# DTUWindEnergy/WindGym

Hardware: AMD Instinct MI355X
Metric: env-steps/sec (whole node), 16-turbine farm x 4096 envs (higher is better)
Workload: dtype f32

## Files before the change

windgym_amd/csrc/wg_api.hip:

```cpp
#include <hip/hip_runtime.h>

#include <algorithm>
#include <cmath>
#include <cstdio>
#include <cstdlib>
#include <cstring>
#include <memory>
#include <mutex>
#include <string>
#include <vector>

#include "wg_plan.h"
#include "wg_steady.h"
#include "wg_policy.h"
#include "wg_internal.h"

static const char* wg_hook(const char* name) {
    static const bool on = [] { const char* v = getenv("WG_DEBUG_HOOKS"); return v && v[0] == '1' && v[1] == 0; }();
    if (!on) return nullptr;
    const char* v = getenv(name);
    if (v) {
        static std::string seen;
        static std::mutex seen_mu;
        std::lock_guard<std::mutex> lock(seen_mu);
        const std::string tag = std::string(name) + "=" + v + ";";
        if (seen.find(tag) == std::string::npos) {
            seen += tag;
            fprintf(stderr, "[windgym] WG_DEBUG_HOOKS: %s=%s\n", name, v);
        }
    }
    return v;
}
static WgHooks wg_hooks_read() {
    WgHooks k;
    const auto num = [](const char* name) { WgHookInt r; if (const char* v = wg_hook(name)) { r.set = true; r.v = atoi(v); } return r; };
    k.flow_block = num("WG_FLOW_BLOCK"); k.flow_res = num("WG_FLOW_RES"); k.flow_env = num("WG_FLOW_ENV");
    k.env_wpe = num("WG_ENV_WPE"); k.env_split = num("WG_ENV_SPLIT"); k.step_fused = num("WG_STEP_FUSED");
    k.sums = num("WG_SUMS"); k.lds_pad = num("WG_LDS_PAD"); k.lf_cap = num("WG_LF_CAP"); k.pstride_pad = num("WG_PSTRIDE_PAD");
    k.step_graph = num("WG_STEP_GRAPH");
    k.first_obs_gl_only = wg_hook("WG_FIRST_OBS_GL_ONLY") != nullptr;
    k.no_box8 = wg_hook("WG_NO_BOX8") != nullptr;
    k.debug = wg_hook("WG_DEBUG") != nullptr;
    if (const char* v = wg_hook("WG_TIMELINE_OUT")) { k.timeline = true; k.timeline_out = v; }
    return k;
}

static thread_local std::string g_err;
static int fail(int code, const std::string& msg) {
    g_err = msg;
    return code;
}
extern "C" int wg_set_last_error_(int code, const char* msg) { return fail(code, msg ? msg : ""); }
#define HIPCHK(x)                                                                                   \
    do {                                                                                            \
        hipError_t _e = (x);                                                                        \
        if (_e != hipSuccess)                                                                       \
            return fail(WG_ERR_HIP, std::string(#x) + ": " + hipGetErrorString(_e));                \
    } while (0)

struct Alloc {
    void* ptr;
    size_t bytes;
};

struct wg_env_s {
    WgPlan plan;
    WgHooks hooks;
    WgParams p;
    WgPtrs d;
    FlowP fp;
    FlowPtrs fd;
    unsigned long long flow_steps_mark = 0, particles_mark = 0, added_mark = 0;
    double added_per_launch = 0.0;
    long n_step_launches = 0;
    void* box4 = nullptr;
    void* box4c = nullptr;
    int* box_ids_dev = nullptr;
    void* abox4 = nullptr;
    void* box8 = nullptr;
    void* abox8 = nullptr;
    double* wind_dev = nullptr;
    int device;
    std::vector<Alloc> allocs;
    std::vector<size_t> state_idx;
    uint8_t* mask_dev = nullptr;
    uint64_t* seeds_dev = nullptr;
    bool timing = false;
    int timing_period = 1, timing_phase = 0;
    std::vector<hipEvent_t> ev;
    std::vector<int> ev_kind;
    size_t ev_used = 0;
    struct StepGraph {
// ... 168 lines not shown
    g.rotor_dy = d.rotor_dy; g.rotor_dz = d.rotor_dz;
    g.gp = h->p_dev; g.gd = h->d_dev; g.env_rw = d.env;
    g.roff = d.roff; g.qown = d.qown; g.status = d.status;
}

static void apply_step_path(wg_env_s* h) {
    wg_plan_step_path(h->plan, h->fp.box_cells, (long long)h->fp.anx * h->fp.any * h->fp.anz, &h->fp.envw, &h->fp.env_fused);
}

extern "C" int wg_create(const wg_config* c, int device, wg_handle* out) {
    if (!c || !out) return fail(WG_ERR_INVALID, "null argument");
    std::string err;
    if (int rc = wg_validate_config(c, &err)) return fail(rc, err);
    HIPCHK(hipSetDevice(device));
    int lds_limit = 65536;
    {
        int v = 0;
        if (hipDeviceGetAttribute(&v, hipDeviceAttributeMaxSharedMemoryPerBlock, device) == hipSuccess && v > 0)
            lds_limit = std::min(v, 65536);
    }
    std::unique_ptr<wg_env_s, HandleGuard> owner(new wg_env_s());
    wg_env_s* h = owner.get();
    h->device = device;
    h->hooks = wg_hooks_read();
    if (int rc = wg_plan_create(c, h->hooks, lds_limit, &h->plan, &err)) return fail(rc, err);
    h->p = h->plan.p;
    h->fp = h->plan.f;
    apply_step_path(h);

    if (int rc = create_alloc(h)) return rc;
    if (int rc = create_upload(h, c)) return rc;
    if (int rc = create_alloc_record(h)) return rc;
    create_flow_ptrs(h);
    if (h->hooks.timeline) {
        long long* dbgp = nullptr;
        if (!dev_alloc(h, &dbgp, (size_t)h->p.B * 2 * h->p.F * 16, false)) h->fd.dbg = dbgp;
    }
    wg_launch_create(&h->p, &h->d, nullptr);
    if (sync_dev_params(h)) return WG_ERR_HIP;
    {
        hipError_t e = hipDeviceSynchronize();
        if (e == hipSuccess) e = hipStreamCreateWithFlags(&h->cap_stream, hipStreamNonBlocking);
        if (e != hipSuccess) return fail(WG_ERR_HIP, std::string("wg_create: ") + hipGetErrorString(e));
    }
    if (h->hooks.step_graph.set) h->graph_mode = h->hooks.step_graph.v != 0;
    if (h->hooks.debug) {
        const FlowP& f = h->fp;
        fprintf(stderr, "[windgym] k_flow variant: %s%s, %d threads, LDS %d B per workgroup, slot stride %d floats\n",
                f.envw ? (f.turb_mode == WG_TURB_NONE ? "compact rings / pair-major, one wave per env (k_flow_env)" : "compact rings / sample-major, one wave per env (k_flow_envb)")
                       : (f.res ? "compact rings / pair-major" : "uniform rings / sample-major"),
                f.envw && f.env_split ? " + a pass wave for the running episode's context" : "",
                f.block, f.envw ? f.env_lds : f.lds_bytes, f.pstride);
        fprintf(stderr, "[windgym] plan: res %d block %d gl %d rec_il %d target_chunk %d lf_cap %d lds_bytes %d | envw %d env_wpe %d env_split %d env_fused %d "
                        "env_lds %d env_off_tab %d | sums_mode %d first_obs %d reset_launches %d\n",
                f.res, f.block, f.gl, f.rec_il, f.target_chunk, f.lf_cap, f.lds_bytes, f.envw, f.env_wpe, f.env_split, f.env_fused, f.env_lds,
                f.env_off_tab, h->p.sums_mode, h->plan.first_obs, h->plan.reset_launches);
    }
    *out = owner.release();
    return 0;
}

extern "C" int wg_destroy(wg_handle h) {
    if (!h) return 0;
    hipSetDevice(h->device);
    hipDeviceSynchronize();
    if (h->fd.dbg && h->hooks.timeline) {
        const size_t n = (size_t)h->p.B * 2 * h->p.F * 16;
        std::vector<long long> host(n);
        if (hipMemcpy(host.data(), h->fd.dbg, n * sizeof(long long), hipMemcpyDeviceToHost) == hipSuccess) {
            if (FILE* f = fopen(h->hooks.timeline_out.c_str(), "wb")) { fwrite(host.data(), sizeof(long long), n, f); fclose(f); }
        }
    }
    drop_step_graphs(h);
    if (h->cap_stream) hipStreamDestroy(h->cap_stream);
    for (auto& e : h->ev) hipEventDestroy(e);
    for (auto& a : h->allocs) hipFree(a.ptr);
    if (h->box4) hipFree(h->box4);
    if (h->box4c) hipFree(h->box4c);
    if (h->abox4) hipFree(h->abox4);
    if (h->box8) hipFree(h->box8);
    if (h->abox8) hipFree(h->abox8);
    delete h;
    return 0;
}

extern "C" int wg_obs_dim(wg_handle h, int* obs_dim, int* obs_dim_multi) {
    if (!h) return fail(WG_ERR_INVALID, "null handle");
    if (obs_dim) *obs_dim = h->p.obs_dim;
    if (obs_dim_multi) *obs_dim_multi = h->p.obs_dim_multi;
    return 0;
}
extern "C" int wg_hist_max(wg_handle h, int* hist_max) {
    if (!h || !hist_max) return fail(WG_ERR_INVALID, "null argument");
    *hist_max = h->p.hist_max;
    return 0;
}

static int build_stencil_records(wg_env_s* h, void** owned, const float4** kernel_ptr, const void* box4, int n_boxes, int nx, int ny, int nz) {
    *kernel_ptr = nullptr;
    if (!(h->fp.envw && h->fp.turb_mode != WG_TURB_NONE)) return 0;
    const auto skip = [h](const char* why) {
        if (h->hooks.debug) fprintf(stderr, "[windgym] stencil records not built (%s): k_flow_envb reads the brick-ordered box\n", why);
        return 0;
    };
    if (wg_hooks_read().no_box8) return skip("WG_NO_BOX8");
    const size_t n_cells = (size_t)nx * ny * nz, bytes = n_cells * 128 * (size_t)n_boxes;
    size_t free_b = 0, total_b = 0;
    if (hipMemGetInfo(&free_b, &total_b) != hipSuccess) return skip("hipMemGetInfo failed");
    if (n_cells >= ((size_t)1 << 28)) return skip("a box of 2^28 cells or more");
// ... 725 lines not shown
```

windgym_amd/csrc/wg_env.hip:

```cpp
#include <hip/hip_runtime.h>

#ifndef WG_ENV_ABLATE
#define WG_ENV_ABLATE 0
#endif
#include "wg_env_common.h"
#include "wg_internal.h"

struct __attribute__((aligned(16))) EnvSlotLds {
    int dev_rem, fill_rem, sub, budget;
    double s_new;
    int n_emit, n_valid, new_valid;
    unsigned n_emitted;
    float s_off_f, near_f, move_max, ti_pow;
    double s_off, ws;
    float ws_f, ti_f, wd_env, base_acc;
    int n_pushed, pend_farm_n, pend_base_n, n_flow;
    double c_time;
    int c_head;
    unsigned c_part, c_flow, c_istep, c_tag, n_emitted0;
    float out_pw;
    unsigned c_add;
    int bg_init;
    int pad_[3];
};
static_assert(sizeof(EnvSlotLds) == WG_ENV_SLOT_LDS_BYTES, "keep WG_ENV_SLOT_LDS_BYTES in sync (wg_flow.h)");
#define WG_ENV_OFF_SRC4 0
#define WG_ENV_OFF_REC4 1024
#define WG_ENV_OFF_RING 2048
#define WG_ENV_OFF_XR 3072
#define WG_ENV_OFF_SRC2 3584
#define WG_ENV_OFF_SL 4096
#define WG_ENV_OFF_HDR (WG_ENV_OFF_SL + 4 * WG_ENV_SLOT_LDS_BYTES)
#define WG_ENV_OFF_STAGE (WG_ENV_OFF_HDR + 128)
static_assert(WG_ENV_OFF_STAGE == WG_ENV_FIXED_LDS_BYTES, "keep WG_ENV_FIXED_LDS_BYTES in sync (wg_flow.h)");

__device__ __forceinline__ float env_slot_sums(const float v, const int N, const int NS, const int k, const int tid) {
    if (N == 16) return wg_row_sum(v);
    if (N < 16) {
        const int r = tid >> 4, i = tid & 15;
        const float x = __shfl(v, (r * N + i) & 63, 64);
        const float s = wg_row_sum((i < N && r < NS) ? x : 0.f);
        return __shfl(s, k << 4, 64);
    }
    const int h = tid >> 5, i = tid & 31;
    const float x = __shfl(v, (h * N + i) & 63, 64);
    float s = (i < N && h < NS) ? x : 0.f;
    WG_ROW_REDUCE(s, wg_addf)
    s += __shfl_xor(s, 16, 64);
    return __shfl(s, k << 5, 64);
}

template <bool NOISE, int WPE, int GLUE, int SPLIT>
__device__ __forceinline__ void env_flow(char* const smem, char* const smem_pass, float* const zone, const int wv, const int role, const int mode,
                                         const float* __restrict__ actions, const uint8_t* __restrict__ mask, const int chunk, EnvFlowOut& out) {
    const int tid = threadIdx.x & 63, e = blockIdx.x;
    int N, F, NS, NL;
    float inv_N;
    {
        const KArgsPtr ka = wg_cold_args();
        N = ka->p.N; F = ka->p.F; inv_N = ka->p.inv_N;
        NS = WPE == 2 ? F : 2 * F; NL = NS * N;
    }
    const int kbase = WPE == 2 ? wv * F : 0;
    const bool valid = tid < NL;
    const int g = valid ? tid : 0;
    const int k = (int)(((float)g + 0.5f) * inv_N);
    const int t = g - k * N;
    const int c = WPE == 2 ? wv : (F == 2 ? (k >> 1) : k), farm = F == 2 ? (k & 1) : 0;

    float4* const Lsrc4 = reinterpret_cast<float4*>(smem + WG_ENV_OFF_SRC4);
    uint4* const Lrec4 = reinterpret_cast<uint4*>(smem + WG_ENV_OFF_REC4);
    int4* const Lring = reinterpret_cast<int4*>(smem + WG_ENV_OFF_RING);
    double* const Lxr = reinterpret_cast<double*>(smem + WG_ENV_OFF_XR);
    float2* const Lsrc2 = reinterpret_cast<float2*>(smem + WG_ENV_OFF_SRC2);
    EnvSlotLds* const SL = reinterpret_cast<EnvSlotLds*>(smem + WG_ENV_OFF_SL);
    float* const def = reinterpret_cast<float*>(smem + WG_ENV_OFF_STAGE);
    float* const tiav = def + WG_ENV_CAP;
    unsigned short* const cl = reinterpret_cast<unsigned short*>(tiav + WG_ENV_CAP);
    unsigned short* const ql = reinterpret_cast<unsigned short*>(smem + WG_ENV_OFF_STAGE);
    EnvSlotLds& my = SL[k];

    WG_STAMP(0);
    typedef const __attribute__((address_space(4))) WgEnv* CEnvPtr;
    int env_live;
    bool role_live = false, role_dev = false, defer_init = false, split_on = false;
    float yaw, tu, tti, oyaw;
    {
        const KArgsPtr k0 = wg_cold_args();
        static_assert(sizeof(WgEnv) == 128, "the env header is loaded as 32 words");
        const int hw = reinterpret_cast<const int*>(k0->d.env + e)[tid & 31];
        if (GLUE != 0 && tid < 32) reinterpret_cast<int*>(smem + WG_ENV_OFF_HDR)[tid] = hw;
        out.bg_init_pending = 0; out.rounds = 0; out.first_obs = 0;
        const bool use_mask = mode == WG_MODE_RESET && mask != nullptr;
        const uint8_t mask_byte = *(use_mask ? mask + e : reinterpret_cast<const uint8_t*>(k0->d.env + e));
        const bool masked_out = use_mask && mask_byte == 0;
        const unsigned ctx_id = (unsigned)(e * 2 + c), slot_id = (unsigned)(e * 2 * F + kbase + k);
        const unsigned tb = (unsigned)((e * 2 * F + kbase) * N + g);
        const unsigned tcx = ctx_id * (unsigned)N + (unsigned)t;

        int dev_rem, fill_rem, n_pushed, pend_farm_n, pend_base_n, init_pending, time_max_c, n_valid, c_head;
        unsigned n_emitted, c_part, c_flow, c_istep, c_tag, c_add;
        double s_off, ws, l_xr, l_yr, c_time;
        float ti_f, wd_env, l_yaw, l_u, l_ti, l_act;
        float4 l_bnd;
        int l_roff, l_rnext;
        auto load_state = [&]() __attribute__((always_inline)) {
            const KArgsPtr kl = wg_cold_args();
            const WgSlot& slot = kl->d.slot[slot_id];
            const WgCtx& cx = kl->d.ctx[ctx_id];
            dev_rem = slot.dev_remaining; fill_rem = slot.fill_remaining;
            s_off = slot.s_off; c_time = slot.time; c_head = slot.head; n_valid = slot.n_valid; c_istep = slot.istep;
            n_emitted = slot.n_emitted; c_part = slot.part_count; c_flow = slot.flow_count; c_add = slot.add_count;
            ws = cx.ws; ti_f = (float)cx.ti; wd_env = (float)cx.wd;
            n_pushed = cx.n_pushed; pend_farm_n = cx.pend_farm_n; pend_base_n = cx.pend_base_n;
            c_tag = (unsigned)cx.episode_tag; init_pending = cx.init_pending; time_max_c = cx.time_max;
            const int* ro = kl->d.roff + ctx_id * (unsigned)(N + 1);
            l_roff = ro[(unsigned)t]; l_rnext = ro[(unsigned)t + 1u];
            l_xr = kl->d.xr[tcx]; l_yr = kl->d.yr[tcx];
            l_yaw = kl->d.yaw[tb]; l_u = kl->d.u[tb]; l_ti = kl->d.ti_loc[tb];
            l_bnd = reinterpret_cast<const float4*>(kl->d.bnd)[tb];
        };
        load_state();
        const int n_tab = k0->p.n_tab, S = k0->p.S;
        const unsigned i_tab = (unsigned)min(tid, n_tab - 1), i_s = (unsigned)min(tid, S - 1);
        const float pf_tp = k0->d.tab_power[i_tab], pf_tc = k0->d.tab_ct[i_tab];
        const float pf_dy = k0->d.rotor_dy[i_s], pf_dz = k0->d.rotor_dz[i_s];
        {
            const bool has_act = mode == WG_MODE_STEP && farm == 0;
            const float a = *(has_act ? actions + (unsigned)(e * N + t) : k0->d.tab_ct);
            l_act = has_act ? a : 0.f;
        }

#define WG_HDR_I(f) __builtin_amdgcn_readlane(hw, (int)(offsetof(WgEnv, f) / 4))
        env_live = WG_HDR_I(live);
        int env_done = WG_HDR_I(done), env_shadow_iters = WG_HDR_I(shadow_iters), env_steps_done = WG_HDR_I(steps_done);
        int env_timestep = WG_HDR_I(timestep), env_time_max_live = WG_HDR_I(time_max_live);
#undef WG_HDR_I
        if (SPLIT && role == 1) {
            if (tid == 0) { *reinterpret_cast<int*>(smem + WG_ENV_OFF_HDR) = 0; if (GLUE != 0 && (SPLIT == 1 || wv == 0)) reinterpret_cast<int*>(zone)[LEAN_PRE_FLAG] = 0; }
            asm volatile("s_waitcnt vmcnt(0) lgkmcnt(0)" ::: "memory");
        }
        if (WPE == 2) {
            asm volatile("" : "+s"(env_live), "+s"(env_done), "+s"(env_shadow_iters), "+s"(env_steps_done), "+s"(env_timestep), "+s"(env_time_max_live) : : "memory");
            asm volatile("s_barrier" ::: "memory");
        }
        if (SPLIT && role == 1 && GLUE != 0 && c == env_live) {
            const EnvKArgsPtr kz = (EnvKArgsPtr)wg_cold_args();
            const WgParams& zp = *(const WgParams*)&kz->gp;
            const WgPtrs& zd = *(const WgPtrs*)&kz->gd;
#define WG_HDR_Z(f) __builtin_amdgcn_readlane(hw, (int)(offsetof(WgEnv, f) / 4))
            const int z_np = WG_HDR_Z(n_pushed_live), z_fn = WG_HDR_Z(farm_pow_n), z_bn = WG_HDR_Z(base_pow_n);
#undef WG_HDR_Z
            const int PA = zp.power_avg;
            const SumsRaw zr = wg_sums_load<false, false>(zp, zd, e, e * 2 + env_live, tid < N ? tid : 0, z_np);
            const float z_fo = zd.farm_pow[(size_t)e * PA + z_fn % PA];
            const float z_bo = F == 2 ? zd.base_pow[(size_t)e * PA + z_bn % PA] : 0.f;
            const float z_met = tid < WG_N_METRICS ? zd.metrics[(size_t)e * WG_N_METRICS + tid] : 0.f;
            double* const zs = reinterpret_cast<double*>(zone);
#pragma unroll
            for (int sI = 0; sI < WG_N_CH; ++sI) { zs[LEAN_PRE_S(sI, tid)] = zr.S[sI]; zone[LEAN_PRE_LV(sI, tid)] = zr.lv[sI]; }
            zone[LEAN_PRE_MET(tid)] = z_met;
            if (tid == 0) { zone[LEAN_PRE_FOLD] = z_fo; zone[LEAN_PRE_BOLD] = z_bo; }
            asm volatile("s_waitcnt lgkmcnt(0)" ::: "memory");
            if (tid == 0) env_flag_set(reinterpret_cast<int*>(zone) + LEAN_PRE_FLAG);
        }
        out.env_live = env_live;
        out.truncates = env_timestep >= env_time_max_live;
        out.steps_done = env_steps_done; out.time_max_live = env_time_max_live;

        const bool is_live_c = (c == env_live);
        const int autoreset = k0->p.autoreset;
        int budget = 0;
        if (mode == WG_MODE_STEP) {
            role_live = is_live_c && !env_done;
            role_dev = !is_live_c && autoreset != 0;
            const int bg_pending = WPE == 2 ? (is_live_c ? 0 : __shfl(init_pending, 0, 64)) : __shfl(init_pending, (env_live ^ 1) * F * N, 64);
            out.bg_init_pending = autoreset && bg_pending;
            if (SPLIT == 2 && role == 1 && out.bg_init_pending) return;
            if (autoreset && bg_pending && WPE == 1 && !out.truncates) {
                defer_init = true;
                budget = 0;
            } else if (autoreset && bg_pending) {
                const KArgsPtr ki = wg_cold_args();
                const WgParams& gp = *ki->d.gp;
                env_init_episode<GLUE != 0>(e, env_live ^ 1, tid);
                full_barrier<64>();
                load_state();
                const int fill_max = F == 2 ? max(gp.fill_a, gp.fill_b) : gp.fill_a;
                const int inc = 1 + (gp.extra_inc ? 1 : 0);
                const int tm = WPE == 2 ? ki->d.ctx[e * 2 + env_live].time_max : __shfl(time_max_c, env_live * F * N, 64);
                const long total = (long)((tm + inc - 1) / inc) + 1;
                const int dev0 = __shfl(dev_rem, WPE == 2 ? 0 : (env_live ^ 1) * F * N, 64);
                budget = wg_shadow_share(dev0 + gp.K * fill_max, total - env_steps_done, env_steps_done, e);
                budget = wg_shadow_share(dev_rem + gp.K * fill_rem, total - env_steps_done, env_steps_done, e, farm ? 0x80000000u : 0u);
            } else {
                const int inc = k0->p.env_inc;
                const long total = (long)((env_time_max_live + inc - 1) / inc) + 1;
                budget = role_dev ? wg_shadow_share(dev_rem + k0->p.K * fill_rem, total - env_steps_done, env_steps_done, e, farm ? 0x80000000u : 0u) : 0;
            }
        } else {
            role_dev = is_live_c && !masked_out;
            budget = chunk;
        }
        if (SPLIT) {
            const bool two = valid && role_dev && budget >= 2;
            split_on = mode == WG_MODE_STEP && k0->p.K == 1 && (is_live_c || (SPLIT == 2 && !out.bg_init_pending)) && !defer_init && !__ballot(two);
            if (role == 1 && !split_on) return;
        }
        if (WPE == 2 && valid && t == 0) {
            my.dev_rem = dev_rem; my.fill_rem = fill_rem; my.bg_init = out.bg_init_pending; my.n_flow = 0; my.out_pw = 0.f;
        }
        {
            const bool any_work = valid && (role_live || (role_dev && budget > 0 && (dev_rem > 0 || fill_rem > 0)));
            if (!__ballot(any_work)) {
                if (WPE == 2 && mode == WG_MODE_STEP && !is_live_c && autoreset && role == 0) {
                    const int d0 = __shfl(dev_rem, 0, 64), f0 = __shfl(fill_rem, 0, 64), np0 = __shfl(n_pushed, 0, 64);
                    const KArgsPtr kf = wg_cold_args();
                    if (d0 == 0 && f0 == 0 && kf->d.gd->next_obs_ok != nullptr && kf->d.gd->next_obs_ok[ctx_id] == 0) {
                        out.first_obs = 1;
                        env_first_obs<GLUE != 0>((int)ctx_id, np0, tid);
                    }
                }
                return;
            }
        }

        const KArgsPtr k1 = wg_cold_args();
        const int rlen = l_rnext - l_roff;
        const int head = n_emitted == 0u ? rlen - 1 : fast_mod((int)(n_emitted - 1u), rlen, __builtin_amdgcn_rcpf((float)rlen));
        const float ws_f = (float)ws;
        if (valid) {
            Lxr[g] = l_xr;
            Lsrc4[g] = make_float4((float)l_xr, (float)l_yr, l_bnd.y, l_bnd.z);
            Lsrc2[g] = make_float2(l_bnd.x, l_bnd.w);
            Lring[g] = make_int4(l_roff, rlen, head, k);
            Lrec4[g] = make_uint4(0u, 0u, 0u, __float_as_uint(1.f));
            if (t == 0) {
                my.dev_rem = dev_rem; my.fill_rem = fill_rem; my.sub = 0; my.budget = budget;
                my.n_valid = n_valid; my.n_emitted = n_emitted; my.n_emitted0 = n_emitted;
                my.move_max = fabsf(k1->p.hill) * ws_f * k1->p.dt; my.ti_pow = fast_pow(ti_f, k1->p.tic);
                my.s_off = s_off; my.ws = ws; my.ws_f = ws_f; my.ti_f = ti_f; my.wd_env = wd_env; my.base_acc = 0.f;
                my.n_pushed = n_pushed; my.pend_farm_n = pend_farm_n; my.pend_base_n = pend_base_n; my.n_flow = 0;
                my.bg_init = out.bg_init_pending;
                my.c_time = c_time; my.c_head = c_head; my.c_part = c_part; my.c_flow = c_flow; my.c_istep = c_istep; my.c_tag = c_tag; my.c_add = c_add;
            }
        }
        float* const tabp = reinterpret_cast<float*>(smem + k1->p.env_off_tab);
        float* const tabct = tabp + n_tab;
        float2* const rpt = reinterpret_cast<float2*>(tabct + n_tab);
        const float hub = k1->p.hub;
        auto rp = [&](const float dy_, const float dz_) __attribute__((always_inline)) {
            const float dz = hub + dz_ - hub;
            return make_float2(dy_, dz * dz);
        };
        if (tid < n_tab) { tabp[tid] = pf_tp; tabct[tid] = pf_tc; }
        if (tid < S) rpt[tid] = rp(pf_dy, pf_dz);
        for (int i = tid + 64; i < n_tab; i += 64) { tabp[i] = k1->d.tab_power[i]; tabct[i] = k1->d.tab_ct[i]; }
        for (int i = tid + 64; i < S; i += 64) rpt[i] = rp(k1->d.rotor_dy[i], k1->d.rotor_dz[i]);

        yaw = l_yaw; tu = l_u; tti = l_ti; oyaw = l_yaw;
        if (role_live && farm == 0 && valid) {
            const float a = l_act, ymin = k1->p.yaw_min, ymax = k1->p.yaw_max, ystep = k1->p.yaw_step;
            if (k1->p.action_method == WG_ACT_YAW) {
                yaw = fminf(fmaxf(yaw + a * ystep, ymin), ymax);
            } else {
                float tf = a + 1.0f;
                tf = tf * 0.5f;
                tf = tf * (ymax - ymin);
                tf = tf + ymin;
                const float ny = fminf(fmaxf(tf, yaw - ystep), yaw + ystep);
                yaw = fminf(fmaxf(ny, ymin), ymax);
            }
        }
    }
    float tpow = 0.f, tct = 0.f, cg = 1.f;
    float sws = 0.f, swd = 0.f, syaw = 0.f, sp_ = 0.f;
    int part_acc = 0, stream_acc = 0;
    bool stepped = false;
    lds_barrier<64>();
    WG_STAMP(1);

    for (int round = 0;; ++round) {
        bool stepping, is_dev;
        int sub, K;
        {
            const KArgsPtr kr = wg_cold_args();
            K = kr->p.K;
            const int4 sch = *reinterpret_cast<const int4*>(&my.dev_rem);
            const bool active = sch.x > 0 || sch.y > 0;
            stepping = valid && (role_live ? (round < K) : (role_dev && active && (sch.w > 0 || sch.z != 0)));
            is_dev = !role_live && sch.x > 0;
            sub = sch.z;
            if (!__ballot(stepping)) break;
        out.rounds = round + 1;
            if (round > 0) full_barrier<64>();

            if (role_live && farm == 1 && stepping) {
                const float ystep = kr->p.yaw_step;
                if (kr->p.base_controller == WG_CTRL_LOCAL) {
                    const float off = 0.f - yaw;
                    const float sgn = (float)((off > 0.f) - (off < 0.f));
                    yaw = yaw + sgn * fminf(fabsf(off), ystep);
                } else {
                    const float sgn = (float)((yaw > 0.f) - (yaw < 0.f));
                    yaw = yaw - sgn * fminf(fabsf(yaw), ystep);
                }
            }

            if (stepping && t == 0) {
                const double dpart = kr->p.dpart;
                const int P = kr->p.P;
                const double s_off = my.s_off, adv = my.ws * kr->p.dt_d;
                double s_new = s_off + adv;
                int n_emit = 0;
                while (s_new >= dpart) { s_new -= dpart; ++n_emit; }
                if (n_emit > P) n_emit = P;
                int new_valid = my.n_valid + n_emit; if (new_valid > P) new_valid = P;
                my.s_new = s_new; my.n_emit = n_emit; my.new_valid = new_valid;
                my.s_off_f = (float)s_off;
                my.near_f = (float)(s_off + adv + dpart) + 0.01f;
            }
        }
        lds_barrier<64>();
        WG_STAMP(4);

        unsigned cmask = 0u;
        {
            const KArgsPtr kp = wg_cold_args();
            const float D = kp->p.D, inv_D = kp->p.inv_D, eps_max = kp->p.env_eps_max;
            const int gs0 = k * N;
            const float lim0 = kp->p.R_rot + 1.0e-3f * D;
            const float near_f = my.near_f, move_max = my.move_max;
            const float xt_f = Lsrc4[g].x, yt_f = Lsrc4[g].y;
#pragma unroll 4
            for (int s2 = 0; s2 < N; ++s2) {
                const float4 a = Lsrc4[gs0 + s2];
                const float2 b = Lsrc2[gs0 + s2];
// ... 623 lines not shown
```

windgym_amd/csrc/wg_flow.h:

```cpp
#pragma once
#include "wg_state.h"

#ifndef WG_BOX_WAVES
#define WG_BOX_WAVES 2
#endif
#ifndef WG_FLOW_WAVES_128
#define WG_FLOW_WAVES_128 6
#endif
#ifndef WG_FLOW_WAVES_CG
#define WG_FLOW_WAVES_CG 5
#endif
#ifndef WG_FLOW_WAVES_GL
#define WG_FLOW_WAVES_GL 4
#endif
#ifndef WG_FLOW_WAVES
#define WG_FLOW_WAVES 5
#endif
#ifndef WG_FLOW_WAVES_LF
#define WG_FLOW_WAVES_LF 3
#endif
#define WG_LF_OFF_TM(n) (16 * (size_t)(n))
#define WG_LF_OFF_BASE(n) (32 * (size_t)(n))
#define WG_LF_OFF_CL(n) ((36 * (size_t)(n) + 4 * 8 + 15) & ~(size_t)15)
#define WG_LF_OFF_DEF(n) ((WG_LF_OFF_CL(n) + (size_t)(n) * ((n) - 1) + 15) & ~(size_t)15)

struct FlowP {
    int B, N, F, K, P, S, S_pad, S_shift, NP, n_tab;
    int autoreset, action_method, base_controller, power_avg, script_rows, noise;
    int block;
    int res;
    int pstride;
    int target_chunk;
    int lf_cap;
    int lds_off_turb, lds_off_tab, lds_bytes;
    int rec_il;
    int gl;
    int lds_off_ql, lds_off_gat;
    int ql_shift;
    int ql_lpt_shift;
    int envw, env_lds, env_off_tab;
    int env_cap, envb_off_cl;
    int env_wpe;
    int env_split;
    int env_fused;
    int env_inc;
    float env_eps_max;
    float dt, D, inv_D, hub, dpart_f, R_rot, inv_N, inv_S, inv_P;
    double dt_d, dpart, inv_dpart;
    float yaw_min, yaw_max, yaw_step;
    float ka, kb, eps0, hill, tia, tib, tic, tid;
    float ue_scale;
    float tab_x0, tab_inv_dx;
    int hlen[WG_N_CH], ring_off[WG_N_CH], fring_off[WG_N_CH];
    float inv_hlen[WG_N_CH], inv_power_avg;
    unsigned hmagic[WG_N_CH], pavg_magic;
    int ring_stride, fring_stride;
    float noise_sigma[WG_N_CH];
    int turb_mode, bnx, bny, bnz, box_pow2;
    int coarse, cnx, cny, cnz, cbox_pow2;
    long long box_cells, cbox_cells;
    double inv_bdx, inv_bdy, inv_bdz, fc_scale, D_d, hub_d;
    float inv_sqrt_S;
    int added, anx, any, anz, abox_pow2;
    int no_ti_fold, deficit_model;
    float km1, km2r;
    float sg_af, sg_bf, sg_cf;
    double inv_adx, inv_ady, inv_adz;
    double inv_bn[3], inv_an[3];
    int an_ct, an_ti, an_x, an_r;
    float an_ct0, an_inv_dct, an_lti0, an_inv_dlti, an_inv_dx, an_inv_dr, an_inv_ka;
};

struct FlowPtrs {
    float *py, *pz, *vlp, *wlp;
    unsigned *rec_a, *rec_b;
    const float4* box4;
    const float4* box4c;
    const float4* abox4;
    const float4* box8;
    const float4* abox8;
    const float* dtab;
    float *yaw, *u, *v, *w, *ti_loc, *power, *ct;
    float* bnd;
    WgSlot* slot;
    WgCtx* ctx;
    const WgEnv* env;
    const double *xr, *yr;
    const int* jneed;
    const int* roff;
    const uint8_t* qown;
    int* status;
    float *ring, *fring, *cur_ws, *cur_wd, *pend_farm, *pend_base, *old_yaw, *step_farm_pow, *step_base_pow;
    const float *rotor_dy, *rotor_dz, *tab_power, *tab_ct;
    const float *script_uvw, *script_power;
    long long* dbg;
    const WgParams* gp;
    const WgPtrs* gd;
    WgEnv* env_rw;
};

// ... 9 lines not shown
```

windgym_amd/csrc/wg_plan.h:

```cpp
#pragma once
#include <algorithm>
#include <cmath>
#include <cstring>
#include <string>
#include <vector>

#ifndef __HIPCC__
struct float4;
#endif
#include "wg_flow.h"

struct WgHookInt {
    bool set = false;
    int v = 0;
};
struct WgHooks {
    WgHookInt flow_block, flow_res, flow_env, env_wpe, env_split, step_fused, sums, lds_pad, lf_cap, pstride_pad, step_graph;
    bool first_obs_gl_only = false, no_box8 = false, debug = false, timeline = false;
    std::string timeline_out;
};

struct WgPlan {
    WgParams p;
    FlowP f;
    int envw_eligible;
    int fused_eligible;
    int first_obs;
    double tab_x0, tab_dx;
    int reset_chunk, reset_launches;
    double alg_bytes;
};

inline double wg_defd(double v, double dflt) { return v == 0.0 ? dflt : v; }

inline int wg_plan_fail(std::string* err, int code, const std::string& msg) {
    if (err) *err = msg;
    return code;
}

inline int wg_validate_config(const wg_config* c, std::string* err) {
    if (!c) return wg_plan_fail(err, WG_ERR_INVALID, "null argument");
    if (c->abi_version != WG_ABI_VERSION) return wg_plan_fail(err, WG_ERR_INVALID, "abi_version mismatch");
    if (c->n_envs < 1 || c->n_turb < 1) return wg_plan_fail(err, WG_ERR_INVALID, "n_envs and n_turb must be >= 1");
    if (c->n_farms != 1 && c->n_farms != 2) return wg_plan_fail(err, WG_ERR_INVALID, "n_farms must be 1 or 2");
    if (c->k_sub < 1) return wg_plan_fail(err, WG_ERR_INVALID, "dt_env must be a multiple of dt_sim");
    if (c->n_particles < 8 || c->n_particles % 4) return wg_plan_fail(err, WG_ERR_INVALID, "n_particles must be a multiple of 4 (>= 8)");
    if (c->n_rotor_pts < 1 || c->n_rotor_pts > 64) return wg_plan_fail(err, WG_ERR_INVALID, "n_rotor_pts must be in [1, 64]");
    if (c->n_turb > 32 * WG_MASK_WORDS) return wg_plan_fail(err, WG_ERR_UNSUPPORTED, "n_turb > 128 is not supported by this build");
    if ((long long)c->n_turb * c->n_particles >= (1ll << 22) || c->n_particles > 16384)
        return wg_plan_fail(err, WG_ERR_UNSUPPORTED, "n_turb * n_particles must stay below 2^22 (and n_particles <= 16384)");
    if (!c->x_pos || !c->y_pos || !c->rotor_dy || !c->rotor_dz || !c->tab_ws || !c->tab_power || !c->tab_ct || c->n_tab < 2)
        return wg_plan_fail(err, WG_ERR_INVALID, "layout / rotor points / turbine table missing");
    if (c->action_method != WG_ACT_YAW && c->action_method != WG_ACT_WIND)
        return wg_plan_fail(err, WG_ERR_UNSUPPORTED, "The ActionMethod must be yaw or wind (absolute is not implemented)");
    if (c->reward_mode < 0 || c->reward_mode > 3)
        return wg_plan_fail(err, WG_ERR_INVALID, "The Power_reward must be either Baseline, Power_avg, None or Power_diff");
    if (c->reward_mode == WG_REW_POWER_DIFF && c->power_avg < 40)
        return wg_plan_fail(err, WG_ERR_INVALID, "The Power_avg must be larger then 40 for the Power_diff reward");
    if (c->reward_mode == WG_REW_BASELINE && c->n_farms != 2)
        return wg_plan_fail(err, WG_ERR_INVALID, "Baseline reward needs the baseline farm (n_farms = 2)");
    if (c->power_avg < 1) return wg_plan_fail(err, WG_ERR_INVALID, "Power_avg must be >= 1");
    if (c->turb_mode < WG_TURB_NONE || c->turb_mode > WG_TURB_BOX_POOL) return wg_plan_fail(err, WG_ERR_INVALID, "Invalid turbulence type specified");
    for (int i = 0; i < WG_N_CH; ++i)
        if (c->ch[i].history_len < 1 || c->ch[i].window_len < 1 || c->ch[i].history_n < 1)
            return wg_plan_fail(err, WG_ERR_INVALID, "sensor history/window lengths must be >= 1");
    {
        const double ka = wg_defd(c->m0_ka, 0.38), kb = wg_defd(c->m0_kb, 0.004), hill = wg_defd(c->m0_hill, 0.4);
        const double tia = c->no_ti_fold ? 0.0 : 0.466 * wg_defd(c->m0_ti_a, 0.73);
        const double k_hi = ka * std::sqrt(c->ti_max * c->ti_max + tia * tia) + kb;
        if (k_hi > 0.25 || std::fabs(hill) * c->ws_max > 16.0)
// ... 245 lines not shown

struct WgEnvbCarve {
    int env_cap, off_cl, off_tab;
    size_t bytes;
};
inline WgEnvbCarve wg_plan_envb_carve(const WgParams& p, int n_tab_u, int wpe) {
    WgEnvbCarve k;
    const int nlp = wpe == 4 ? 16 : 64;
    const int nl_w = (wpe == 4 ? 1 : (wpe == 2 ? p.F : 2 * p.F)) * p.N;
    k.env_cap = wpe == 4 ? 128 : 256;
    size_t ob = WG_ENVB_FIXED_LDS_BYTES(nlp) + (size_t)20 * k.env_cap;
    k.off_cl = (int)ob;
    ob = (ob + (size_t)2 * nl_w * (p.N > 1 ? p.N - 1 : 1) + 15) & ~(size_t)15;
    k.off_tab = (int)ob;
    ob += sizeof(float) * (2 * (size_t)n_tab_u + 2 * (size_t)p.S);
    k.bytes = (ob + 15) & ~(size_t)15;
    return k;
}

inline bool wg_plan_envb(const WgParams& p, const WgHooks& hk, FlowP& f, bool small, int lds_limit, int* wpe) {
    const int NL = 2 * p.F * p.N;
    *wpe = (p.B <= 2048) ? 2 : 1;
    if (hk.env_wpe.set) {
        const int w = hk.env_wpe.v;
        *wpe = (w == 4 && p.F == 2 && p.N <= 16) ? 4 : (w == 2 ? 2 : (w == 4 ? 2 : 1));
    }
    if (!(f.res && small && f.block == 64 && !f.gl && p.turb_mode >= WG_TURB_BOX && NL <= 64 && p.N <= 32 && p.P <= 4096 && f.S_pad <= 16 &&
          f.deficit_model == 0))
        return false;
    WgEnvbCarve k = wg_plan_envb_carve(p, f.n_tab, *wpe);
    while (*wpe > 1 && *wpe * k.bytes + 64 > (size_t)lds_limit) {
        *wpe /= 2;
        k = wg_plan_envb_carve(p, f.n_tab, *wpe);
    }
    f.env_cap = k.env_cap; f.envb_off_cl = k.off_cl; f.env_off_tab = k.off_tab; f.env_lds = (int)k.bytes;
    return f.env_lds <= 32768 && f.env_lds <= lds_limit;
}

inline void wg_plan_step_kernels(const wg_config* c, const WgHooks& hk, const WgParams& p, FlowP& f, bool small, int lds_limit) {
    const size_t qf = wg_plan_farm_quads(c, p);
    const bool env_ok = wg_plan_env(p, f, small, qf, lds_limit);
    int envb_wpe = 1;
    const bool envb_ok = wg_plan_envb(p, hk, f, small, lds_limit, &envb_wpe);
    f.env_inc = 1 + (p.extra_inc ? 1 : 0);
    f.env_eps_max = std::min(1.0f, (float)(p.eps0 * std::sqrt(3.0))) + 2.0f / 65535.0f;
    f.envw = ((env_ok || envb_ok) && !hk.flow_block.set && !hk.flow_res.set) ? 1 : 0;
    if (hk.flow_env.set) f.envw = ((env_ok || envb_ok) && hk.flow_env.v != 0) ? 1 : 0;
    f.env_wpe = (p.B <= 2048 && 2 * f.env_lds <= lds_limit) ? 2 : 1;
    if (hk.env_wpe.set) f.env_wpe = (hk.env_wpe.v == 2 && 2 * f.env_lds <= lds_limit) ? 2 : 1;
    const bool split_ok = env_ok && f.env_wpe == 2 && p.K == 1 && 4 * f.env_lds + 4096 <= lds_limit;
    f.env_split = (split_ok && p.B <= 1024 && qf >= 256) ? (p.B <= 512 ? 2 : 1) : 0;
    if (hk.env_split.set) f.env_split = (hk.env_split.v != 0 && split_ok && p.B <= 2048) ? (hk.env_split.v == 2 ? 2 : 1) : 0;
    if (envb_ok) f.env_wpe = envb_wpe;
    const bool gen = p.turb_ti || p.farm_ti || p.farm_obs > 0 || (p.sum_mask_f | p.cur_mask_f) != 0;
    f.env_fused = (f.envw && p.sums_mode && !gen && p.power_avg <= 64) ? 1 : 0;
    if (hk.step_fused.set) f.env_fused = (f.env_fused && hk.step_fused.v != 0) ? 1 : 0;
}

inline void wg_plan_flow_scalars(const wg_config* c, const WgParams& p, double tab_x0, double tab_dx, FlowP& f) {
    f.B = p.B; f.N = p.N; f.F = p.F; f.K = p.K; f.P = p.P; f.S = p.S; f.NP = p.NP;
    f.S_pad = 1; f.S_shift = 0;
    while (f.S_pad < p.S) { f.S_pad <<= 1; f.S_shift++; }
    f.autoreset = p.autoreset; f.action_method = p.action_method; f.base_controller = p.base_controller;
    f.power_avg = p.power_avg; f.script_rows = 0; f.noise = (p.noise == WG_NOISE_NORMAL);
    f.dt = p.dt; f.D = p.D; f.inv_D = p.inv_D; f.hub = p.hub; f.dpart_f = (float)p.dpart; f.R_rot = 0.5f * p.D;
    f.inv_N = 1.0f / (float)p.N; f.inv_S = 1.0f / (float)p.S; f.inv_P = 1.0f / (float)p.P;
    f.inv_power_avg = 1.0f / (float)(p.power_avg > 0 ? p.power_avg : 1);
    f.pavg_magic = (unsigned)((1ull << 32) / (unsigned long long)(p.power_avg > 0 ? p.power_avg : 1)) + 1u;
    f.dt_d = p.dt_d; f.dpart = p.dpart; f.inv_dpart = 1.0 / p.dpart;
    f.yaw_min = p.yaw_min; f.yaw_max = p.yaw_max; f.yaw_step = p.yaw_step;
    f.ka = p.ka; f.kb = p.kb; f.eps0 = p.eps0; f.hill = p.hill; f.tia = p.tia; f.tib = p.tib; f.tic = p.tic; f.tid = p.tid;
    f.tab_x0 = (float)tab_x0; f.tab_inv_dx = (float)(1.0 / tab_dx);
    f.ue_scale = p.turb_mode == WG_TURB_NONE ? 1.0f : 2.0f;
    for (int i = 0; i < WG_N_CH; ++i) {
        f.hlen[i] = p.ring_cap[i]; f.ring_off[i] = p.ring_off[i]; f.fring_off[i] = p.fring_off[i];
        f.inv_hlen[i] = 1.0f / (float)p.ring_cap[i];
        f.hmagic[i] = (unsigned)((1ull << 32) / (unsigned long long)p.ring_cap[i]) + 1u;
        f.noise_sigma[i] = p.noise_sigma[i];
    }
    f.ring_stride = p.ring_stride; f.fring_stride = p.fring_stride;
    f.turb_mode = p.turb_mode; f.fc_scale = p.fc_scale; f.D_d = p.D_d; f.hub_d = p.hub_d;
    f.inv_sqrt_S = 1.0f / std::sqrt((float)p.S);
    f.added = (c->added_turbulence != 0 && c->turb_mode != WG_TURB_NONE) ? 1 : 0;
    f.no_ti_fold = c->no_ti_fold != 0; f.deficit_model = c->deficit_model;
    f.km1 = (float)wg_defd(c->m0_km1, 0.6); f.km2r = (float)(2.0 * wg_defd(c->m0_km2, 0.35) * 0.5 * p.D_d);
    f.sg_af = (float)wg_defd(c->m0_sg_af, 3.11); f.sg_bf = (float)wg_defd(c->m0_sg_bf, -0.68); f.sg_cf = (float)wg_defd(c->m0_sg_cf, 2.41);
    f.an_inv_ka = (float)(1.0 / wg_defd(c->m0_ka, 0.38));
}

inline int wg_plan_reset_launches(const wg_config* c, const WgParams& p, int reset_chunk) {
    double xmn = 1e300, xmx = -1e300, ymn = 1e300, ymx = -1e300;
    for (int t = 0; t < p.N; ++t) {
        xmn = std::min(xmn, c->x_pos[t]); xmx = std::max(xmx, c->x_pos[t]);
        ymn = std::min(ymn, c->y_pos[t]); ymx = std::max(ymx, c->y_pos[t]);
    }
    const double ext_x = xmx - xmn, ext_y = ymx - ymn;
    const double diag = std::sqrt(ext_x * ext_x + ext_y * ext_y);
    const double ws_lo = std::max(1e-3, std::min(c->ws_min, c->ws_max));
    const long max_dev = (long)std::ceil(2.0 * diag / ws_lo / c->dt_sim) + 2;
    const long max_work = max_dev + (long)p.K * (std::max(p.fill_a, p.fill_b) + 1);
    return (int)((max_work + reset_chunk - 1) / reset_chunk) + 1;
}

inline double wg_plan_alg_bytes(const WgParams& p) {
    const bool turb = p.turb_mode != WG_TURB_NONE, boxm = p.turb_mode >= WG_TURB_BOX;
    const double per_farm_step = (double)p.NP * (4 + 4 + 8 + (turb ? 24 : 0) + (boxm ? 64 : 0)) +
// ... 50 lines not shown
```

Measured before the change: 82.78 million.

## Share background-episode development between twin farms by cloning lead farm state

When two farms per env both need to develop a fresh background episode, the second farm is parked and, once the first finishes development, its particle/record state, LDS slots and turbine outputs are copied from the twin instead of being simulated again. The lead farm's budget is widened to cover the twin's fill, and split mode is disabled when a clone is pending. This removes duplicated flow simulation during autoreset development, at the cost of extra global copies, barriers and added control complexity.

```diff
diff --git a/windgym_amd/csrc/wg_api.hip b/windgym_amd/csrc/wg_api.hip
--- a/windgym_amd/csrc/wg_api.hip
+++ b/windgym_amd/csrc/wg_api.hip
@@ -37,7 +37,7 @@
     k.flow_block = num("WG_FLOW_BLOCK"); k.flow_res = num("WG_FLOW_RES"); k.flow_env = num("WG_FLOW_ENV");
     k.env_wpe = num("WG_ENV_WPE"); k.env_split = num("WG_ENV_SPLIT"); k.step_fused = num("WG_STEP_FUSED");
     k.sums = num("WG_SUMS"); k.lds_pad = num("WG_LDS_PAD"); k.lf_cap = num("WG_LF_CAP"); k.pstride_pad = num("WG_PSTRIDE_PAD");
-    k.step_graph = num("WG_STEP_GRAPH");
+    k.step_graph = num("WG_STEP_GRAPH"); k.share_dev = num("WG_ENV_SHARE_DEV");
     k.first_obs_gl_only = wg_hook("WG_FIRST_OBS_GL_ONLY") != nullptr;
     k.no_box8 = wg_hook("WG_NO_BOX8") != nullptr;
     k.debug = wg_hook("WG_DEBUG") != nullptr;
@@ -312,9 +312,9 @@
                 f.envw && f.env_split ? " + a pass wave for the running episode's context" : "",
                 f.block, f.envw ? f.env_lds : f.lds_bytes, f.pstride);
         fprintf(stderr, "[windgym] plan: res %d block %d gl %d rec_il %d target_chunk %d lf_cap %d lds_bytes %d | envw %d env_wpe %d env_split %d env_fused %d "
-                        "env_lds %d env_off_tab %d | sums_mode %d first_obs %d reset_launches %d\n",
-                f.res, f.block, f.gl, f.rec_il, f.target_chunk, f.lf_cap, f.lds_bytes, f.envw, f.env_wpe, f.env_split, f.env_fused, f.env_lds,
-                f.env_off_tab, h->p.sums_mode, h->plan.first_obs, h->plan.reset_launches);
+                        "env_share %d env_lds %d env_off_tab %d | sums_mode %d first_obs %d reset_launches %d\n",
+                f.res, f.block, f.gl, f.rec_il, f.target_chunk, f.lf_cap, f.lds_bytes, f.envw, f.env_wpe, f.env_split, f.env_fused, f.env_share,
+                f.env_lds, f.env_off_tab, h->p.sums_mode, h->plan.first_obs, h->plan.reset_launches);
     }
     *out = owner.release();
     return 0;
diff --git a/windgym_amd/csrc/wg_env.hip b/windgym_amd/csrc/wg_env.hip
--- a/windgym_amd/csrc/wg_env.hip
+++ b/windgym_amd/csrc/wg_env.hip
@@ -50,6 +50,48 @@
     return __shfl(s, k << 5, 64);
 }
 
+static __device__ __forceinline__ void env_clone_dev(char* const smem, const int kd, const int N, const int P, const double dt_d,
+                                                               float* const py_env, unsigned* const ra_env, const unsigned src,
+                                                               const unsigned dst, const int lane) {
+    float4* const Lsrc4 = reinterpret_cast<float4*>(smem + WG_ENV_OFF_SRC4);
+    int4* const Lring = reinterpret_cast<int4*>(smem + WG_ENV_OFF_RING);
+    float2* const Lsrc2 = reinterpret_cast<float2*>(smem + WG_ENV_OFF_SRC2);
+    EnvSlotLds* const SL = reinterpret_cast<EnvSlotLds*>(smem + WG_ENV_OFF_SL);
+    const int ga = (kd - 1) * N, gb = kd * N;
+    const int4 last = Lring[ga + N - 1];
+    const int nq = (last.x + last.y) >> 2;
+    {
+        const float4* const ps = reinterpret_cast<const float4*>(py_env + src);
+        float4* const pd = reinterpret_cast<float4*>(py_env + dst);
+        const uint4* const rs = reinterpret_cast<const uint4*>(ra_env + 2 * (size_t)src);
+        uint4* const rd = reinterpret_cast<uint4*>(ra_env + 2 * (size_t)dst);
+#pragma unroll 2
+        for (int q = lane; q < nq; q += 64) {
+            const float4 y = ps[q];
+            const uint4 r0 = rs[q], r1 = rs[q + nq];
+            pd[q] = y; rd[q] = r0; rd[q + nq] = r1;
+        }
+    }
+    if (lane < N) {
+        Lsrc4[gb + lane] = Lsrc4[ga + lane];
+        Lsrc2[gb + lane] = Lsrc2[ga + lane];
+        Lring[gb + lane].z = Lring[ga + lane].z;
+    }
+    if (lane == 0) {
+        const EnvSlotLds& a = SL[kd - 1];
+        EnvSlotLds& b = SL[kd];
+        b.n_valid = a.n_valid; b.n_emitted = a.n_emitted; b.s_off = a.s_off;
+        b.dev_rem = 0; b.sub = 0;
+        b.budget = a.budget;
+        double tm = a.c_time;
+        for (int i = 0; i < a.n_flow; ++i) tm += dt_d;
+        b.c_time = tm;
+        int hd = a.c_head + (int)((a.n_emitted - a.n_emitted0) % (unsigned)P); if (hd >= P) hd -= P;
+        b.c_head = hd; b.n_emitted0 = a.n_emitted;
+        b.c_istep = a.c_istep + (unsigned)a.n_flow;
+    }
+}
+
 template <bool NOISE, int WPE, int GLUE, int SPLIT>
 __device__ __forceinline__ void env_flow(char* const smem, char* const smem_pass, float* const zone, const int wv, const int role, const int mode,
                                          const float* __restrict__ actions, const uint8_t* __restrict__ mask, const int chunk, EnvFlowOut& out) {
@@ -84,6 +126,7 @@
     typedef const __attribute__((address_space(4))) WgEnv* CEnvPtr;
     int env_live;
     bool role_live = false, role_dev = false, defer_init = false, split_on = false;
+    bool parked = false;
     float yaw, tu, tti, oyaw;
     {
         const KArgsPtr k0 = wg_cold_args();
@@ -171,6 +214,7 @@
         const bool is_live_c = (c == env_live);
         const int autoreset = k0->p.autoreset;
         int budget = 0;
+        long plan_left = 0;
         if (mode == WG_MODE_STEP) {
             role_live = is_live_c && !env_done;
             role_dev = !is_live_c && autoreset != 0;
@@ -193,18 +237,32 @@
                 const int dev0 = __shfl(dev_rem, WPE == 2 ? 0 : (env_live ^ 1) * F * N, 64);
                 budget = wg_shadow_share(dev0 + gp.K * fill_max, total - env_steps_done, env_steps_done, e);
                 budget = wg_shadow_share(dev_rem + gp.K * fill_rem, total - env_steps_done, env_steps_done, e, farm ? 0x80000000u : 0u);
+                plan_left = total - env_steps_done;
             } else {
                 const int inc = k0->p.env_inc;
                 const long total = (long)((env_time_max_live + inc - 1) / inc) + 1;
                 budget = role_dev ? wg_shadow_share(dev_rem + k0->p.K * fill_rem, total - env_steps_done, env_steps_done, e, farm ? 0x80000000u : 0u) : 0;
+                plan_left = total - env_steps_done;
             }
         } else {
             role_dev = is_live_c && !masked_out;
             budget = chunk;
         }
+        bool clone_here = false;
+        if (k0->p.env_share) {
+            const int dev_a = __shfl(dev_rem, (tid - N) & 63, 64);
+            parked = valid && role_dev && farm == 1 && dev_rem > 0 && c_istep == 0u && dev_a > 0;
+            const int twin_fill = __shfl(parked ? fill_rem + 1 : 0, (tid + N) & 63, 64);
+            const bool lead = valid && role_dev && farm == 0 && twin_fill > 0;
+            if (lead && mode == WG_MODE_STEP && !defer_init)
+                budget = wg_shadow_share(dev_rem + k0->p.K * max(fill_rem, twin_fill - 1), plan_left, env_steps_done, e);
+            if (parked) budget = 0;
+            clone_here = lead && budget >= dev_rem;
+        }
         if (SPLIT) {
             const bool two = valid && role_dev && budget >= 2;
-            split_on = mode == WG_MODE_STEP && k0->p.K == 1 && (is_live_c || (SPLIT == 2 && !out.bg_init_pending)) && !defer_init && !__ballot(two);
+            split_on = mode == WG_MODE_STEP && k0->p.K == 1 && (is_live_c || (SPLIT == 2 && !out.bg_init_pending)) && !defer_init && !__ballot(two) &&
+                       !__ballot(clone_here);
             if (role == 1 && !split_on) return;
         }
         if (WPE == 2 && valid && t == 0) {
@@ -283,6 +341,27 @@
     for (int round = 0;; ++round) {
         bool stepping, is_dev;
         int sub, K;
+        if (__ballot(parked)) {
+            bool due = parked && SL[k - 1].dev_rem == 0;
+            unsigned long long due_m = __ballot(due);
+            if (due_m) {
+                full_barrier<64>();
+                const KArgsPtr kc = wg_cold_args();
+                const unsigned pstride = (unsigned)kc->p.pstride;
+                const size_t pb_env = (size_t)(e * 2 * F + kbase) * pstride;
+                const int src_lane = (tid - N) & 63;
+                const float c_tu = __shfl(tu, src_lane, 64), c_tti = __shfl(tti, src_lane, 64), c_pw = __shfl(tpow, src_lane, 64);
+                const float c_ct = __shfl(tct, src_lane, 64), c_cg = __shfl(cg, src_lane, 64);
+                if (due) { tu = c_tu; tti = c_tti; tpow = c_pw; tct = c_ct; cg = c_cg; stepped = true; parked = false; }
+                while (due_m) {
+                    const int kd = __builtin_amdgcn_readlane(k, __builtin_ctzll(due_m));
+                    env_clone_dev(smem, kd, N, kc->p.P, kc->p.dt_d, kc->d.py + pb_env, kc->d.rec_a + 2 * pb_env, (unsigned)(kd - 1) * pstride,
+                                  (unsigned)kd * pstride, tid);
+                    due_m &= ~(((1ull << N) - 1ull) << (kd * N));
+                }
+                lds_barrier<64>();
+            }
+        }
         {
             const KArgsPtr kr = wg_cold_args();
             K = kr->p.K;
diff --git a/windgym_amd/csrc/wg_flow.h b/windgym_amd/csrc/wg_flow.h
--- a/windgym_amd/csrc/wg_flow.h
+++ b/windgym_amd/csrc/wg_flow.h
@@ -46,6 +46,7 @@
     int env_inc;
     float env_eps_max;
     float dt, D, inv_D, hub, dpart_f, R_rot, inv_N, inv_S, inv_P;
+    int env_share;
     double dt_d, dpart, inv_dpart;
     float yaw_min, yaw_max, yaw_step;
     float ka, kb, eps0, hill, tia, tib, tic, tid;
diff --git a/windgym_amd/csrc/wg_plan.h b/windgym_amd/csrc/wg_plan.h
--- a/windgym_amd/csrc/wg_plan.h
+++ b/windgym_amd/csrc/wg_plan.h
@@ -15,7 +15,7 @@
     int v = 0;
 };
 struct WgHooks {
-    WgHookInt flow_block, flow_res, flow_env, env_wpe, env_split, step_fused, sums, lds_pad, lf_cap, pstride_pad, step_graph;
+    WgHookInt flow_block, flow_res, flow_env, env_wpe, env_split, step_fused, sums, lds_pad, lf_cap, pstride_pad, step_graph, share_dev;
     bool first_obs_gl_only = false, no_box8 = false, debug = false, timeline = false;
     std::string timeline_out;
 };
@@ -367,6 +367,8 @@
     f.env_split = (split_ok && p.B <= 1024 && qf >= 256) ? (p.B <= 512 ? 2 : 1) : 0;
     if (hk.env_split.set) f.env_split = (hk.env_split.v != 0 && split_ok && p.B <= 2048) ? (hk.env_split.v == 2 ? 2 : 1) : 0;
     if (envb_ok) f.env_wpe = envb_wpe;
+    f.env_share = (f.envw && env_ok && p.F == 2) ? 1 : 0;
+    if (hk.share_dev.set && hk.share_dev.v == 0) f.env_share = 0;
     const bool gen = p.turb_ti || p.farm_ti || p.farm_obs > 0 || (p.sum_mask_f | p.cur_mask_f) != 0;
     f.env_fused = (f.envw && p.sums_mode && !gen && p.power_avg <= 64) ? 1 : 0;
     if (hk.step_fused.set) f.env_fused = (f.env_fused && hk.step_fused.v != 0) ? 1 : 0;
```

Result: faster. 89.52 million, median of 6 (+8.1%).
